# paulffm/Continuous-Time-Diffusion-Models-for-Discrete-Data

Measured on AMD Instinct MI355X. Metric: tau-leaping sample-steps/s, higher is better.
Workload: dtype bf16; 1 GPU; MNIST tauLDR U-Net TauL step (config_tauUnet_mnist: D=784, S=256, 1000-step grid); batch_per_gpu=256, global_batch=256, D=784, S=256, parallelism=sample-sharded x1, no collective in the loop

## Files before the change

### continuous-time-diffusion-models-for-discrete-data_amd/ctdd/native.py

```python
import ctypes as C
import os

import torch

_HERE = os.path.dirname(os.path.dirname(os.path.abspath(__file__)))
_LIB = None

BRANCH_CTELBO, BRANCH_CRM = 0, 1
LOGIT_TYPES = {"direct": 0, "reverse_prob": 1, "reverse_logscale": 2}
STEP_ORDINAL, STEP_CORRECTOR, STEP_COUNT_RAW, STEP_CRM, STEP_COUNT_JUMPS, STEP_BF16, STEP_LOGITS_BF16 = 1, 2, 4, 8, 16, 32, 64


class CtddError(RuntimeError):
    pass


def lib_path():
    return os.environ.get("CTDD_LIBRARY") or os.path.join(_HERE, "libctdd.so")


_P, _I, _F, _U64, _U32, _I64 = C.c_void_p, C.c_int, C.c_float, C.c_uint64, C.c_uint32, C.c_int64
_SIGS = {
    "ctdd_abi_version": ([], _I),
    "ctdd_last_error": ([], C.c_char_p),
    "ctdd_rate_table": ([_P, _P, _P, _P, _P, _P, _I, _I, _I, _F, _P, _P, _P, _P, _P], _I),
    "ctdd_noise_categorical": ([_P, _P, _P, _P, _U64, _U64, _I, _I, _I, _P, _P], _I),
    "ctdd_xtilde_sample": ([_P, _P, _P, _P, _P, _U64, _U64, _I, _I, _I, _P, _P, _P, _P], _I),
    "ctdd_xtilde_sample_masked": ([_P, _P, _P, _P, _P, _P, _U64, _U64, _I, _I, _I, _P, _P, _P, _P], _I),
    "ctdd_logprob": ([_P, _P, _P, _P, _I, _I, _I, _I, _P, _P, _P], _I),
    "ctdd_reverse_rates": ([_I, _I, _P, _P, _P, _P, _P, _F, _I, _I, _I, _P, _P, _P], _I),
    "ctdd_tauleap_apply": ([_P, _P, _P, _I, _I, _I, _I, _P, _P, _P], _I),
    "ctdd_tauleap_draw": ([_P, _P, _P, _F, _U32, _U64, _U64, _I, _I, _I, _P, _P, _P], _I),
    "ctdd_tauleap_step": ([_I, _I, _P, _P, _P, _P, _P, _F, _F, _F, _U32, _U64, _U64, _I, _I, _I, _P, _P, _P], _I),
    "ctdd_tauleap_step_rows": ([_I, _I, _P, _P, _P, _P, _P, _F, _F, _F, _U32, _U64, _U64, _I, _I, _I, _P, _I, _P, _P, _P], _I),
    "ctdd_lbjf_step": ([_I, _I, _P, _P, _P, _P, _F, _F, _F, _U32, _P, _U64, _U64, _I, _I, _I, _P, _P, _P, _P], _I),
    "ctdd_logprob_rp_mfma": ([_P, _P, _P, _I, _I, _I, _P, _P, _P, _P], _I),
    "ctdd_logprob_rp_bwd_mfma": ([_P, _P, _P, _P, _P, _F, _I, _I, _I, _P, _P, _P, _P, _P], _I),
    "ctdd_exact_step": ([_P, _P, _P, _P, _P, _U64, _U64, _I, _I, _I, _P, _P, _P, _P], _I),
    "ctdd_midpoint_predict": ([_I, _I, _P, _P, _P, _P, _F, _F, _F, _I, _I, _I, _P, _P], _I),
    "ctdd_lbjf_from_rates": ([_P, _P, _F, _P, _U64, _U64, _I, _I, _I, _P, _P, _P, _P], _I),
    "ctdd_midpoint_from_rates": ([_P, _P, _F, _I, _I, _I, _P, _P], _I),
    "ctdd_lbjf_step_rows": ([_I, _I, _P, _P, _P, _P, _F, _F, _F, _U32, _P, _U64, _U64, _I, _I, _I, _P, _I, _P, _P, _P, _P], _I),
    "ctdd_midpoint_predict_rows": ([_I, _I, _P, _P, _P, _P, _F, _F, _F, _I, _I, _I, _P, _I, _P, _P], _I),
    "ctdd_exact_step_rows": ([_P, _P, _P, _P, _P, _U64, _U64, _I, _I, _I, _P, _I, _P, _P, _P, _P], _I),
    "ctdd_lbjf_from_rates_rows": ([_P, _P, _F, _P, _U64, _U64, _I, _I, _I, _P, _I, _P, _P, _P, _P], _I),
    "ctdd_midpoint_from_rates_rows": ([_P, _P, _F, _I, _I, _I, _P, _I, _P, _P], _I),
    "ctdd_argmax": ([_P, _I, _I, _I, _P, _P], _I),
    "ctdd_initial_samples": ([_P, _U64, _U64, _I, _I, _I, _P, _P], _I),
    "ctdd_philox_uniform": ([_U64, _U64, _I64, _I, _P, _P], _I),
    "ctdd_s256_step_table_bytes": ([], _I64),
    "ctdd_s256_prepare": ([_P, _P, _F, _I, _P, _P, _P, _P], _I),
    "ctdd_s256_prepare_crm": ([_P, _P, _I, _P, _P, _P, _P], _I),
    "ctdd_tauleap_step_s256": ([_P, _P, _P, _P, _P, _P, _F, _F, _U32, _U64, _U64, _I, _I, _P, _P, _P, _P], _I),
    "ctdd_tauleap_step_s256_rows": ([_P, _P, _P, _P, _P, _P, _F, _F, _U32, _U64, _U64, _I, _I, _P, _I, _P, _P, _P, _P], _I),
    "ctdd_crm_loss": ([_P, _P, _P, _P, _I, _I, _I, _I, _F, _F, _P, _P, _P, _P], _I),
    "ctdd_ctelbo_scratch_bytes": ([_I, _I, _I], _I64),
    "ctdd_ctelbo_loss": ([_P, _P, _P, _P, _P, _P, _I, _I, _I, _F, _F, _F, _P, _P, _P, _P], _I),
    "ctdd_ctelbo_loss_terms": ([_P, _P, _P, _P, _P, _P, _I, _I, _I, _F, _F, _F, _F, _P, _P, _P, _P], _I),
    "ctdd_ctelbo_loss_window": ([_P, _P, _P, _P, _P, _P, _I, _I, _I, _I, _I, _F, _F, _F, _F, _P, _P, _P, _P], _I),
    "ctdd_ctelbo_loss_masked": ([_P, _P, _P, _P, _P, _P, _P, _I, _I, _I, _F, _F, _F, _F, _P, _P, _P, _P], _I),
    "ctdd_score_elbo_loss": ([_P, _P, _P, _P, _P, _P, _I, _I, _I, _F, _F, _P, _P, _P, _P], _I),
    "ctdd_crm_loss_ll": ([_P, _P, _P, _I, _I, _I, _I, _F, _P, _P, _P, _P], _I),
    "ctdd_score_elbo_loss_ll": ([_P, _P, _P, _P, _P, _P, _I, _I, _I, _F, _F, _P, _P, _P, _P], _I),
    "ctdd_logprob_bwd": ([_I, _P, _P, _P, _P, _P, _F, _I, _I, _I, _P, _P, _P, _P], _I),
    "ctdd_crm_loss_masked": ([_P, _P, _P, _P, _P, _I, _I, _I, _I, _F, _F, _P, _P, _P, _P], _I),
    "ctdd_crm_loss_ll_masked": ([_P, _P, _P, _P, _I, _I, _I, _I, _F, _P, _P, _P, _P], _I),
    "ctdd_score_elbo_loss_masked": ([_P, _P, _P, _P, _P, _P, _P, _I, _I, _I, _F, _F, _P, _P, _P, _P], _I),
    "ctdd_score_elbo_loss_ll_masked": ([_P, _P, _P, _P, _P, _P, _P, _I, _I, _I, _F, _F, _P, _P, _P, _P], _I),
    "ctdd_opt_chunk_elems": ([], _I),
    "ctdd_adam_ema_step": ([_P, _P, _I, _F, _F, _F, _F, _I64, _F, _F, _P, _P], _I),
    "ctdd_grad_sumsq": ([_P, _P, _I, _P, _I, _P], _I),
    "ctdd_adam_ema_apply": ([_P, _P, _I, _F, _F, _F, _F, _I64, _F, _F, _P, _P], _I),
}
UNET_EXPORTS = ("ctdd_unet_conv", "ctdd_unet_conv_patch", "ctdd_unet_conv_res", "ctdd_unet_conv_ring", "ctdd_unet_conv_up_phases", "ctdd_unet_upsample2x", "ctdd_unet_first_conv", "ctdd_unet_gn_apply", "ctdd_unet_gn_onepass", "ctdd_unet_channel_stats",
                "ctdd_unet_time", "ctdd_unet_time_uniform", "ctdd_unet_attention", "ctdd_unet_logistic_head", "ctdd_unet_resblock_small",
                "ctdd_unet_resblock_mid", "ctdd_unet_conv_rows")
HOLLOW_EXPORTS = ("ctdd_gemm_bf16", "ctdd_hollow_small_linear", "ctdd_hollow_embed", "ctdd_hollow_layernorm", "ctdd_hollow_add", "ctdd_hollow_put_rows", "ctdd_hollow_attention", "ctdd_hollow_attention_bf16")
UNET_TRAIN_EXPORTS = ("ctdd_unet_wgrad", "ctdd_unet_gn_bwd", "ctdd_unet_dropout", "ctdd_unet_colsum", "ctdd_unet_sum_batch", "ctdd_unet_sum_jobs", "ctdd_unet_accumulate",
                      "ctdd_unet_downsum2x", "ctdd_unet_upsample2x_f32", "ctdd_unet_cast_rows", "ctdd_unet_attention_bwd",
                      "ctdd_unet_first_conv_wgrad", "ctdd_unet_first_conv_wgrad_scratch", "ctdd_unet_pack_weights",
                      "ctdd_unet_unpack_grads")
HOLLOW_TRAIN_EXPORTS = ("ctdd_hollow_layernorm_bwd", "ctdd_hollow_attention_train", "ctdd_hollow_attention_bwd", "ctdd_hollow_attention_train_bf16", "ctdd_hollow_attention_bwd_bf16", "ctdd_hollow_act", "ctdd_hollow_relu_bf16", "ctdd_hollow_colsum", "ctdd_hollow_dropout",
                        "ctdd_hollow_embed_bwd")
BERT_EXPORTS = ("ctdd_bert_embed", "ctdd_bert_gather", "ctdd_bert_attention_short",
                "ctdd_bert_embed_bwd", "ctdd_bert_gather_bwd",
                "ctdd_bert_embed_enum_bwd", "ctdd_bert_gather_enum_bwd",
                "ctdd_bert_attention_short_train", "ctdd_bert_attention_short_bwd")
EXPORTS = tuple(_SIGS) + UNET_EXPORTS + HOLLOW_EXPORTS + UNET_TRAIN_EXPORTS + HOLLOW_TRAIN_EXPORTS + BERT_EXPORTS


def load():
    global _LIB
    if _LIB is None:
        path = lib_path()
        if not os.path.exists(path):
            raise CtddError(f"{path} not found: build it with `python __graft_entry__.py` "
                            "(hipcc --offload-arch=gfx950); there is no CPU fallback")
        lib = C.CDLL(path)
        for name, (argt, rest) in _SIGS.items():
            fn = getattr(lib, name)
            fn.argtypes, fn.restype = argt, rest
        _LIB = lib
    return _LIB


def _ptr(t, dtype=None, name="tensor"):
    if t is None:
        return None
    if not isinstance(t, torch.Tensor):
        raise CtddError(f"{name}: expected a torch tensor, got {type(t)}")
    if not t.is_cuda:
        raise CtddError(f"{name}: must live on a GPU (got {t.device}); libctdd has no CPU path")
    if dtype is not None and t.dtype != dtype:
        raise CtddError(f"{name}: expected {dtype}, got {t.dtype}")
    if not t.is_contiguous():
        raise CtddError(f"{name}: must be contiguous")
    return t.data_ptr()


def _stream():
    return torch.cuda.current_stream().cuda_stream


def _check(rc, what):
    if rc != 0:
        msg = load().ctdd_last_error().decode(errors="replace")
        raise CtddError(f"{what} failed with status {rc}: {msg}")


# ... 607 lines not shown
```

### continuous-time-diffusion-models-for-discrete-data_amd/ctdd/unet_engine.py

```python
import contextlib
import ctypes as C

import torch

from . import native
from .plan_launch import bound_launch, graph_capture, ptr

_P, _I, _F = C.c_void_p, C.c_int, C.c_float
SEG_3x3, SEG_1x1, SEG_3x3_S2, SEG_3x3_UP = 0, 1, 2, 3


class _Seg(C.Structure):
    _fields_ = [("hi", _P), ("f32", _P), ("C", _I), ("kind", _I)]


class _ConvArgs(C.Structure):
    _fields_ = [("seg", _Seg * 3), ("nseg", _I), ("w_hi", _P), ("w_f32", _P), ("B", _I), ("H", _I), ("W", _I),
                ("Hin", _I), ("Win", _I), ("N", _I), ("Ktot", _I), ("bias", _P), ("tbias", _P), ("tb_stride", _I),
                ("res_f32", _P), ("res_bf16", _P), ("out_f32", _P), ("out_hi", _P), ("stats", _P), ("logits_C", _I),
                ("ksplit", _I), ("acc_buf", _P), ("act", _I), ("out_lo", _P)]


class _FirstArgs(C.Structure):
    _fields_ = [("x64", _P), ("x32", _P), ("lo", _F), ("hi", _F), ("w", _P), ("bias", _P), ("B", _I), ("Cin", _I),
                ("H", _I), ("W", _I), ("Cout", _I), ("out_f32", _P), ("out_hi", _P), ("stats", _P), ("x0_f32", _P)]


class _GnArgs(C.Structure):
    _fields_ = [("s1_f32", _P), ("s1_bf16", _P), ("st1", _P), ("C1", _I), ("s2_f32", _P), ("s2_bf16", _P), ("st2", _P),
                ("C2", _I), ("gamma", _P), ("beta", _P), ("B", _I), ("HW", _I), ("G", _I), ("eps", _F), ("swish", _I),
                ("out_hi", _P), ("out_f32", _P)]


class _ResblockArgs(C.Structure):
    _fields_ = [("s1_bf16", _P), ("s2_bf16", _P), ("C1", _I), ("C2", _I), ("gamma1", _P), ("beta1", _P), ("gamma2", _P), ("beta2", _P),
                ("G1", _I), ("G2", _I), ("eps1", _F), ("eps2", _F), ("w1", _P), ("bias1", _P), ("tbias", _P), ("tb_stride", _I),
                ("w2", _P), ("bias2", _P), ("skip", _I), ("B", _I), ("H", _I), ("W", _I), ("N", _I), ("out_bf16", _P)]


class _ConvRowsArgs(C.Structure):
    _fields_ = [("s1_bf16", _P), ("st1", _P), ("C1", _I), ("s2_bf16", _P), ("st2", _P), ("C2", _I), ("gamma", _P), ("beta", _P), ("G", _I),
                ("eps", _F), ("w", _P), ("bias", _P), ("tbias", _P), ("tb_stride", _I), ("r1_bf16", _P), ("RC1", _I), ("r2_bf16", _P),
                ("RC2", _I), ("res_bf16", _P), ("out_bf16", _P), ("out_stats", _P), ("B", _I), ("H", _I), ("W", _I), ("N", _I)]


class _TimeArgs(C.Structure):
    _fields_ = [("t", _P), ("B", _I), ("ch", _I), ("tdim", _I), ("w1", _P), ("b1", _P), ("w2", _P), ("b2", _P),
                ("hid", _P), ("act", _P)]


class _AttnArgs(C.Structure):
    _fields_ = [("qkv", _P), ("B", _I), ("T", _I), ("C", _I), ("heads", _I), ("out_hi", _P), ("out_f32", _P)]


class _LogisticArgs(C.Structure):
    _fields_ = [("net", _P), ("x0", _P), ("B", _I), ("C", _I), ("HW", _I), ("S", _I), ("fix", _I), ("out", _P), ("fast", _I), ("out_bf16", _P)]


_sigs_done = False


def _lib():
    global _sigs_done
    lib = native.load()
    if not _sigs_done:
        for name, argt in (("ctdd_unet_conv", [_P, _I, _I, _I, _P]), ("ctdd_unet_conv_patch", [_P, _I, _I, _I, _P]), ("ctdd_unet_conv_res", [_P, _I, _P]), ("ctdd_unet_conv_ring", [_P, _I, _P]),
                           ("ctdd_unet_conv_up_phases", [_P, _I, _P]), ("ctdd_unet_upsample2x", [_P, _I, _I, _I, _I, _P, _P]), ("ctdd_unet_first_conv", [_P, _P]),
                           ("ctdd_unet_gn_apply", [_P, _P]), ("ctdd_unet_gn_onepass", [_P, _I, _I, _P]), ("ctdd_unet_channel_stats", [_P, _I, _I, _I, _P, _P]),
                           ("ctdd_unet_time", [_P, _P, _P, _I, _P, _P]), ("ctdd_unet_time_uniform", [_P, _P, _P, _I, _P, _P]),
                           ("ctdd_unet_attention", [_P, _P]), ("ctdd_unet_resblock_small", [_P, _I, _P]),
                           ("ctdd_unet_resblock_mid", [_P, _I, _P]), ("ctdd_unet_conv_rows", [_P, _I, _P]),
                           ("ctdd_unet_logistic_head", [_P, _P])):
            fn = getattr(lib, name)
            fn.argtypes, fn.restype = argt, _I
        _sigs_done = True
    return lib


def _unwrap(net):
    return net.module if hasattr(net, "module") and net.__class__.__name__ == "DistributedDataParallel" else net


def supports(model):
    net = _unwrap(getattr(model, "net", None))
    return (net is not None and net.__class__.__name__ == "UNet" and not model.padding
            and model.cfg.model.model_output in ("logits", "logistic_pars"))


def training_supported(model):
    if getattr(model.cfg.model, "engine_train", "hip") != "hip" or not supports(model):
        return False
    net = _unwrap(model.net)
    return net.channel % 16 == 0 and all((net.channel * int(m_)) % 16 == 0 for m_ in model.cfg.model.ch_mult)



def resblock_small_covers(H, W, cs, cout, G1, G2):
    Ct = sum(cs)
    if H * W > 64 or W > 8 or cout != 192 or len(cs) > 2 or any(c % 64 for c in cs) or Ct > 384 or Ct % G1 or cout % G2:
        return False
    if H * W > 16 and (H - 1) * (W + 2) + W > 80:
        return False
    rs_a, rs_2, prows = Ct * 2 + 32, cout * 2 + 32, (H + 2) * (W + 2)
    return H * W * rs_a + prows * max(rs_a, rs_2) + 256 * 80 + 2 * 384 * 8 + 2 * 384 * 4 <= 160 * 1024


def pack_resblock_weights(w2d):
    N, K = w2d.shape
    assert N == 192 and K % 64 == 0
    return w2d.reshape(4, 3, 16, K // 64, 2, 4, 8).permute(0, 3, 1, 4, 5, 2, 6).contiguous().reshape(N, K)


def resblock_mid_covers(H, W, cs, cout, G1, G2):
    Ct = sum(cs)
    if (H < 1 or W < 1 or H > 14 or W > 14 or cout != 192 or not 1 <= len(cs) <= 2
            or any(c <= 0 or c % 32 or c > 192 for c in cs) or G1 <= 0 or G2 <= 0 or Ct % G1 or cout % G2):
        return False
    return ((H + 2) * 16 + 2) * (cout * 2 + 32) + 256 * 80 + 2 * 384 * 8 + 2 * 384 * 4 <= 160 * 1024


def pack_row_tile_weights(w, cs, rcs, streams):
    N, Ct, Rt = w.shape[0], sum(cs), sum(rcs)
    assert N == 48 * streams and w.shape[1] == 9 * Ct + Rt and all(c % 32 == 0 for c in [*cs, *rcs])
    w3, parts, c0 = w[:, :9 * Ct].reshape(N, 9, Ct), [], 0
    for c in cs:
        v = w3[:, :, c0:c0 + c].reshape(streams, 3, 16, 3, 3, c // 32, 4, 8)
        parts.append(v.permute(0, 5, 4, 3, 1, 6, 2, 7).reshape(streams, -1))
        c0 += c
    c0 = 9 * Ct
    for c in rcs:
        v = w[:, c0:c0 + c].reshape(streams, 3, 16, c // 32, 4, 8)
        parts.append(v.permute(0, 3, 1, 4, 2, 5).reshape(streams, -1))
        c0 += c
    return torch.cat(parts, 1).contiguous().reshape(N, w.shape[1])


def pack_resblock_mid_weights(w1, w2, cs):
    N = w1.shape[0]
    return pack_row_tile_weights(w1, cs, [], 4), pack_row_tile_weights(w2, [N], cs if w2.shape[1] > 9 * N else [], 4)


def pack_conv_rows_weights(w, cs, rcs):
    return pack_row_tile_weights(w, cs, rcs, 2)


CONV_ROWS_MIN_WGS = 96


def conv_rows_covers(H, W, cs, rcs, cout, G, residual=False):
    return bool(H >= 1 and 1 <= W <= 28 and cout == 96 and 1 <= len(cs) <= 2 and len(rcs) <= 2 and all(c > 0 and c % 32 == 0 for c in [*cs, *rcs])
                and sum(cs) <= 384 and sum(rcs) <= 384 and G > 0 and sum(cs) % G == 0 and not (rcs and residual))


def fold_upsample_weights(w):
    N, Cn = w.shape[:2]
    assert tuple(w.shape[2:]) == (3, 3)
    sel = torch.tensor([[[1, 0, 0], [0, 1, 1]], [[1, 1, 0], [0, 0, 1]]], dtype=w.dtype, device=w.device)
    return torch.einsum("pia,qjb,ncab->pqnijc", sel, sel, w).reshape(4, N, 4 * Cn).contiguous()


def upsample_phases_covers(B, Hs, Ws, Cn, N):
    return bool(Cn >= 16 and Cn % 16 == 0 and (N % 96 == 0 or N % 64 == 0) and N > 0 and 1 <= Ws <= 33 and Hs * Ws >= 32
                and 4 * Cn * 64 < 2 ** 31 and 4 * B * Hs * Ws < 2 ** 31)


def _onepass_slab(B, HW, Cn, G, max_threads=1024):
    if Cn % 8 or G <= 0 or Cn % G:
        return 0
    cg = Cn // G
    L = cg
    while L % 8:
        L += cg
    best = 0
    for sc in range(L, Cn + 1, L):
        if Cn % sc:
            continue
        noct = sc // 8
        if noct > max_threads:
            continue
        npl = min(max_threads // noct, HW)
        if -(-HW // npl) > 12:
            continue
        wgs = B * (Cn // sc)
        if best == 0 or wgs >= 256:
            best = sc
        if wgs < 256:
            break
    return best


class _Tensor:

    def __init__(self, pb, H, W, Cn, stats=True):
        eng, B = pb.eng, pb.B
        M = B * H * W
        self.B, self.H, self.W, self.C = B, H, W, Cn
        self.f32 = torch.empty((M, Cn), dtype=torch.float32, device=eng.dev) if eng.precise else None
        self.hi = None if eng.precise else torch.empty((M, Cn), dtype=torch.bfloat16, device=eng.dev)
        small = H * W <= pb.no_stats_hw
        self.stats_by_gn = bool(stats and small and pb.gn_writes_stats)
        self.stats = pb.alloc_stats(B * Cn * 2) if (stats and (not small or self.stats_by_gn)) else None
        pb.keep.append(self)


# ... 160 lines not shown
        s1 = srcs[0]
        a.s1_f32, a.s1_bf16, a.C1 = (ptr(s1.f32), None, s1.C) if eng.precise else (None, ptr(s1.hi), s1.C)
        if s1.stats is not None:
            self.stats_views.append((a, s1.stats, "st1"))
        if len(srcs) == 2:
            s2 = srcs[1]
            a.s2_f32, a.s2_bf16, a.C2 = (ptr(s2.f32), None, s2.C) if eng.precise else (None, ptr(s2.hi), s2.C)
            if s2.stats is not None:
                self.stats_views.append((a, s2.stats, "st2"))
        g, b_ = norm.weight.detach().float().contiguous(), norm.bias.detach().float().contiguous()
        self.keep.extend([g, b_, a, out])
        a.gamma, a.beta = ptr(g), ptr(b_)
        a.B, a.HW, a.G, a.eps, a.swish = B, HW, norm.num_groups, eps, int(swish)
        a.out_hi, a.out_f32 = ptr(out.hi), ptr(out.f32)
        if self.onepass_gn and HW <= self.no_stats_hw:
            if _onepass_slab(B, HW, Ct, norm.num_groups, self.gn_threads) == 0:
                raise native.CtddError(f"one-pass GroupNorm does not cover HW={HW} C={Ct} G={norm.num_groups}")
            self.launch(lib.ctdd_unet_gn_onepass, C.byref(a), 0, self.gn_threads, label=f"gn1 {srcs[0].H}x{srcs[0].W} C={Ct} ({len(srcs)} src)")
        else:
            self.launch(lib.ctdd_unet_gn_apply, C.byref(a), label=f"gn {srcs[0].H}x{srcs[0].W} C={Ct} ({len(srcs)} src)")
        if tc is not None:
            tc.record_gn(self, srcs, norm, swish, eps, HW, out, drop_p)
        return out

    def conv_rows(self, srcs, norm, segs, wsrc, bias, out, tb=None, res=None, raws=()):
        eng, lib, B = self.eng, self.lib, self.B
        Hc, Wc, N = srcs[0].H, srcs[0].W, out.C
        cs, rcs = [s_.C for s_ in srcs], [s_.C for s_ in raws]
        a = _ConvRowsArgs()
        for i, s_ in enumerate(srcs):
            setattr(a, f"s{i + 1}_bf16", ptr(s_.hi))
            setattr(a, f"C{i + 1}", s_.C)
            self.stats_views.append((a, s_.stats, f"st{i + 1}"))
        for i, s_ in enumerate(raws):
            setattr(a, f"r{i + 1}_bf16", ptr(s_.hi))
            setattr(a, f"RC{i + 1}", s_.C)
        g, b_ = norm.weight.detach().float().contiguous(), norm.bias.detach().float().contiguous()
        a.gamma, a.beta, a.G, a.eps = ptr(g), ptr(b_), norm.num_groups, norm.eps
        w, _ = eng._pack(pack_conv_rows_weights(eng._w2d(wsrc, segs), cs, rcs))
        a.w, a.bias = ptr(w), ptr(bias)
        if tb is not None:
            a.tbias, a.tb_stride = tb
        if res is not None:
            a.res_bf16 = ptr(res.hi)
        a.out_bf16 = ptr(out.hi)
        if out.stats is not None and not out.stats_by_gn:
            self.stats_views.append((a, out.stats, "out_stats"))
        a.B, a.H, a.W, a.N = B, Hc, Wc, N
        self.keep.extend([g, b_, w, bias, a])
        Ktot = w.shape[1]
        self.launch(lib.ctdd_unet_conv_rows, C.byref(a), 0, label=f"{Hc}x{Wc} K={Ktot} N={N} gn+conv rows C={cs} raw={rcs}",
                    flops=2 * B * Hc * Wc * N * Ktot)

    def conv2_operands(self, rb, a2, srcs):
        tc = self.tc
        segs, wsrc, bias_params = [(a2, rb.conv2.weight.shape[0], SEG_3x3)], [(rb.conv2.weight, 0)], [rb.conv2.bias]
        bias = rb.conv2.bias.detach().float()
        if rb.skip is not None:
            c_ = 0
            for s_ in srcs:
                segs.append((s_, s_.C, SEG_1x1))
                wsrc.append((rb.skip.weight, c_))
                c_ += s_.C
            bias_params.append(rb.skip.bias)
            bias = tc.summed_bias(bias_params) if tc is not None else bias + rb.skip.bias.detach().float()
        return segs, wsrc, bias_params, bias.contiguous()

    def resblock_fused(self, rb, srcs, mid=False):
        eng, lib, B = self.eng, self.lib, self.B
        Hc, Wc = srcs[0].H, srcs[0].W
        cs = [s.C for s in srcs]
        Ct, cout = sum(cs), rb.conv1.weight.shape[0]
        y = _Tensor(self, Hc, Wc, cout)
        a = _ResblockArgs()
        a.s1_bf16, a.C1 = ptr(srcs[0].hi), cs[0]
        if len(srcs) == 2:
            a.s2_bf16, a.C2 = ptr(srcs[1].hi), cs[1]
        par = [p_.detach().float().contiguous() for p_ in (rb.norm1.weight, rb.norm1.bias, rb.norm2.weight, rb.norm2.bias, rb.conv1.bias)]
        a.gamma1, a.beta1, a.gamma2, a.beta2, a.bias1 = (ptr(p_) for p_ in par)
        a.G1, a.G2, a.eps1, a.eps2 = rb.norm1.num_groups, rb.norm2.num_groups, rb.norm1.eps, rb.norm2.eps
        a.tbias, a.tb_stride = self.tproj.data_ptr() + 4 * self.toff[id(rb)], self.tb_stride
        w1 = eng._w2d([(rb.conv1.weight, 0)], [(None, Ct, SEG_3x3)])
        segs, wsrc, _, bias2 = self.conv2_operands(rb, None, srcs)
        w2 = eng._w2d(wsrc, segs)
        w1, w2 = pack_resblock_mid_weights(w1, w2, cs) if mid else (pack_resblock_weights(w1), pack_resblock_weights(w2))
        (w1, _), (w2, _) = eng._pack(w1), eng._pack(w2)
        a.w1, a.w2, a.bias2, a.skip = ptr(w1), ptr(w2), ptr(bias2), int(rb.skip is not None)
        a.B, a.H, a.W, a.N, a.out_bf16 = B, Hc, Wc, cout, ptr(y.hi)
        self.keep.extend(par + [w1, w2, bias2, a])
        K1, K2 = w1.shape[1], w2.shape[1]
        self.launch(lib.ctdd_unet_resblock_mid if mid else lib.ctdd_unet_resblock_small, C.byref(a), 0,
                    label=f"{Hc}x{Wc} resblock C={cs} N={cout} K={K1}+{K2}", flops=2 * B * Hc * Wc * cout * (9 * Ct + 9 * cout + (Ct if rb.skip is not None else 0)))
        return y

    def resblock(self, rb, srcs):
        eng, tc = self.eng, self.tc
        Hc, Wc = srcs[0].H, srcs[0].W
        cs = [s.C for s in srcs]
        cout = rb.conv1.weight.shape[0]
        if self.onepass_gn and eng._fuses_resblock(rb, Hc, Wc, cs, tc is not None) and all(s_.stats is None for s_ in srcs):
            return self.resblock_fused(rb, srcs)
        if self.onepass_gn and eng._fuses_resblock_mid(rb, Hc, Wc, cs, tc is not None) and all(s_.stats is None for s_ in srcs):
            return self.resblock_fused(rb, srcs, mid=True)
        tbias = (self.tproj.data_ptr() + 4 * self.toff[id(rb)], self.tb_stride)
        h = _Tensor(self, Hc, Wc, cout)
        b1 = rb.conv1.bias.detach().float().contiguous()
# ... 96 lines not shown
        self.conv([(cur, cur.C, SEG_3x3_S2)], [(cv.weight, 0)],
                  cv.bias.detach().float().contiguous(), cur.C, Ho, Wo, cur.H, cur.W, y, bias_params=[cv.bias])
        return y

    def upsample_in_phases(self, cur):
        eng, m, B, Cn = self.eng, self.m, self.B, cur.C
        if self.tc is not None or eng.precise or not int(getattr(m, "upsample_phases", 1)):
            return False
        Ho, Wo = cur.H * 2, cur.W * 2
        ring = self.pick_kernel(True, B * Ho * Wo, Cn, Ho, Wo) == "ring" and Wo <= 33 and Cn % 32 == 0
        if not ring or (getattr(m, "conv_ksplit", 1) > 1 and Cn // 16 >= 2) or getattr(m, "ring_small_tiles", 0):
            return False
        return upsample_phases_covers(B, cur.H, cur.W, Cn, Cn)

    def upsample_phases(self, cv, cur, y):
        eng, B, Cn = self.eng, self.B, cur.C
        a = _ConvArgs()
        a.nseg = 1
        a.seg[0].hi, a.seg[0].C, a.seg[0].kind = ptr(cur.hi), Cn, SEG_3x3_UP
        whi, _ = eng._pack(fold_upsample_weights(cv.weight.detach().float()).reshape(4 * Cn, 4 * Cn))
        bias = cv.bias.detach().float().contiguous()
        a.w_hi, a.bias = ptr(whi), ptr(bias)
        a.B, a.H, a.W, a.Hin, a.Win, a.N, a.Ktot = B, y.H, y.W, cur.H, cur.W, Cn, 4 * Cn
        a.out_hi = ptr(y.hi)
        if y.stats is not None and not y.stats_by_gn:
            self.stats_views.append((a, y.stats, "stats"))
        self.keep.extend([whi, bias, a])
        self.launch(self.lib.ctdd_unet_conv_up_phases, C.byref(a), 0, label=f"{y.H}x{y.W} K=4x{4 * Cn} N={Cn} up-phases of {cur.H}x{cur.W}",
                    flops=2 * B * y.H * y.W * Cn * 4 * Cn)

    def upsample(self, cv, cur):
        eng, tc, B, lib = self.eng, self.tc, self.B, self.lib
        y = _Tensor(self, cur.H * 2, cur.W * 2, cur.C)
        if self.upsample_in_phases(cur):
            self.upsample_phases(cv, cur, y)
        elif eng.precise and tc is None:
            self.conv([(cur, cur.C, SEG_3x3_UP)], [(cv.weight, 0)],
                      cv.bias.detach().float().contiguous(), cur.C, cur.H * 2, cur.W * 2, cur.H, cur.W, y)
        else:
            up = _Tensor(self, cur.H * 2, cur.W * 2, cur.C, stats=False)
            if eng.precise:
                self.launch(lib.ctdd_unet_upsample2x_f32, ptr(cur.f32), B, cur.H, cur.W, cur.C, ptr(up.f32))
            else:
                self.launch(lib.ctdd_unet_upsample2x, ptr(cur.hi), B, cur.H, cur.W, cur.C, ptr(up.hi))
            if tc is not None:
                tc.record_upsample(cur, up)
            self.conv([(up, cur.C, SEG_3x3)], [(cv.weight, 0)],
                      cv.bias.detach().float().contiguous(), cur.C, up.H, up.W, up.H, up.W, y, bias_params=[cv.bias])
        return y

    def head(self, cur, logits_out, logits_bf16):
        eng, tc, B, st, m, net, dev, (Cin, H0, W0) = self.eng, self.tc, self.B, self.st, self.m, self.net, self.dev, self.shape
        S = net.S
        ao = self.gn_apply([cur], net.out[0], True, net.out[0].eps, cur.H * cur.W)
        oc = net.out[2]
        n_out = oc.weight.shape[0]
        D = Cin * H0 * W0
        logistic = m.model_output == "logistic_pars"
        ldt = torch.bfloat16 if logits_bf16 and not (logistic and (tc is not None or eng.precise or S % 4)) else torch.float32
        st.logits = logits_out if logits_out is not None else torch.empty((B, D, S), dtype=ldt, device=dev)
        assert st.logits.dtype == ldt
        if logistic:
            st.net_out = torch.empty((B * H0 * W0, n_out), dtype=torch.float32, device=dev)
            self.conv([(ao, ao.C, SEG_3x3)], [(oc.weight, 0)],
                      oc.bias.detach().float().contiguous(), n_out, H0, W0, H0, W0, None, out_f32_tensor=st.net_out, bias_params=[oc.bias])
            la = _LogisticArgs()
            la.net, la.x0, la.B, la.C, la.HW, la.S, la.fix = ptr(st.net_out), ptr(st.x0), B, Cin, H0 * W0, S, int(bool(m.fix_logistic))
            if ldt == torch.bfloat16:
                la.out_bf16 = ptr(st.logits)
            else:
                la.out = ptr(st.logits)
            la.fast = 0 if eng.precise else 1
            self.keep.append(la)
            if tc is None:
                self.launch(self.lib.ctdd_unet_logistic_head, C.byref(la))
        else:
            self.conv([(ao, ao.C, SEG_3x3)], [(oc.weight, 0)],
                      oc.bias.detach().float().contiguous(), n_out, H0, W0, H0, W0, None, out_f32_tensor=st.logits,
                      logits_C=Cin, bias_params=[oc.bias])

    def build(self, x_dtype, logits_out, logits_bf16, uniform_t):
        st, B, net, dev = self.st, self.B, self.net, self.dev
        st.x_in = torch.zeros((B, *self.shape), dtype=x_dtype, device=dev)
        st.t_in = torch.zeros((B,), dtype=torch.float32, device=dev)
        self.time(uniform_t)
        cur = self.first_conv(net.down[0])
        feats = [cur]
        for layer in list(net.down)[1:]:
            cur = self.block(layer, [cur]) if hasattr(layer, "resblocks") else self.downsample(layer.downsample[0], cur)
            feats.append(cur)
        for layer in net.mid:
            cur = self.block(layer, [cur])
        for layer in net.up:
            cur = self.block(layer, [cur, feats.pop()]) if hasattr(layer, "resblocks") else self.upsample(layer[1], cur)
        self.head(cur, logits_out, logits_bf16)
        if self.tc is not None:
            self.tc.finish(self)
        st.stats = torch.zeros((max(self.stats_off, 1),), dtype=torch.float64, device=dev)
        base = st.stats.data_ptr()
        for a_, off, field in self.stats_views:
            setattr(a_, field, base + 8 * off)
        nz = sum(n for _, n in self.zero_views)
        st.zpool = torch.zeros((max(nz, 1),), dtype=torch.float32, device=dev)
        zo = 0
        for a_, n in self.zero_views:
            a_.acc_buf = st.zpool.data_ptr() + 4 * zo
            zo += n
        st.plan, st.keep, st.graph = self.plan, self.keep, None
        return st


class UNetEngine:
    def __init__(self, model, precision=None):
        self.model = model
# ... 11 lines not shown
        self._time_w = None

    def _weights_version(self):
        return sum(p._version for p in self.net.parameters()) + 7919 * getattr(self.model, "_weights_version", 0)

    def _pack(self, w2d):
        w = w2d.detach().float().contiguous()
        return (None, w) if self.precise else (w.to(torch.bfloat16).contiguous(), None)

    @staticmethod
    def _w2d(wsrc, segs):
        parts = []
        for (w, c_off), (_, cs, kind) in zip(wsrc, segs):
            w = w.detach().float()
            N = w.shape[0]
            if kind == SEG_1x1:
                parts.append(w.reshape(N, -1)[:, c_off:c_off + cs])
            else:
                parts.append(w[:, c_off:c_off + cs].permute(0, 2, 3, 1).reshape(N, 9 * cs))
        return torch.cat(parts, dim=1).contiguous()


    def _time_weights(self):
        ver = self._weights_version()
        if self._time_w is None or self._time_w[0] != ver:
            net = self.net
            resblocks = [mod.resblocks for mod in list(net.down) + list(net.mid) + list(net.up) if hasattr(mod, "resblocks")]
            pw = torch.cat([rb.time[1].weight.detach().float() for rb in resblocks], 0).t().contiguous()
            pb = torch.cat([rb.time[1].bias.detach().float() for rb in resblocks], 0).contiguous()
            tw = [net.time[1].weight.t(), net.time[1].bias, net.time[3].weight.t(), net.time[3].bias]
            tw = [w.detach().float().contiguous() for w in tw]
            self._time_w = (ver, resblocks, pw, pb, tw)
        return self._time_w[1:]

    def _onepass_max_hw(self):
        return int(getattr(self.cfg.model, "gn_onepass_max_hw", 256))

    def _fuses_resblock(self, rb, Hc, Wc, cs, training):
        return bool(not training and not self.precise and int(getattr(self.cfg.model, "resblock_fused", 1))
                    and Hc * Wc <= self._onepass_max_hw()
                    and resblock_small_covers(Hc, Wc, cs, rb.conv1.weight.shape[0], rb.norm1.num_groups, rb.norm2.num_groups))

    def _fuses_resblock_mid(self, rb, Hc, Wc, cs, training):
        return bool(not training and not self.precise and int(getattr(self.cfg.model, "resblock_fused_mid", 1))
                    and Hc * Wc <= self._onepass_max_hw()
                    and not resblock_small_covers(Hc, Wc, cs, rb.conv1.weight.shape[0], rb.norm1.num_groups, rb.norm2.num_groups)
                    and resblock_mid_covers(Hc, Wc, cs, rb.conv1.weight.shape[0], rb.norm1.num_groups, rb.norm2.num_groups))

    def _runs_conv_rows(self, B, Hc, Wc, cs, rcs, cout, G, residual, training):
        m = self.cfg.model
        return bool(not training and not self.precise and int(getattr(m, "conv_rows", 1))
                    and conv_rows_covers(Hc, Wc, cs, rcs, cout, G, residual)
                    and B * -(-Hc // 14) >= int(getattr(m, "conv_rows_min_wgs", CONV_ROWS_MIN_WGS)))

    def _onepass_gn_covers(self, B, training):
        net, (_, H, W) = self.net, self.cfg.data.shape
        max_hw, threads = self._onepass_max_hw(), int(getattr(self.cfg.model, "gn_threads", 512))
        norms, c = [], net.channel
        for layer in [*list(net.down)[1:], *net.mid, *net.up]:
            if hasattr(layer, "downsample"):
                H, W = (H + 1 - 3) // 2 + 1, (W + 1 - 3) // 2 + 1
            elif not hasattr(layer, "resblocks"):
                H, W = 2 * H, 2 * W
            else:
                rb, c1 = layer.resblocks, layer.resblocks.norm1.num_channels
                cs = [c] if c1 == c else [c, c1 - c]
                if not (self._fuses_resblock(rb, H, W, cs, training) or self._fuses_resblock_mid(rb, H, W, cs, training)):
                    norms += [(H * W, rb.norm1), (H * W, rb.norm2)]
                c = rb.norm2.num_channels
                if layer.attention is not None:
                    norms.append((H * W, layer.attention.norm))
        norms.append((H * W, net.out[0]))
        return all(hw > max_hw or _onepass_slab(B, hw, n.num_channels, n.num_groups, threads) > 0 for hw, n in norms)

    def _build(self, B, x_dtype, logits_out=None, tc=None, logits_bf16=False, uniform_t=False):
        m = self.cfg.model
        onepass_gn = bool((not self.precise) and int(getattr(m, "gn_onepass", 1)) and (tc is None or int(getattr(m, "gn_onepass_train", 1)))
                          and self._onepass_gn_covers(B, tc is not None))
        return _PlanBuilder(self, B, tc, onepass_gn).build(x_dtype, logits_out, logits_bf16, uniform_t)

    def _run_plan(self, st):
        st.stats.zero_()
        st.zpool.zero_()
        for step in st.plan:
            step()

    def _prepare(self, B, x_dtype, x, times, logits_out=None, logits_bf16=False, uniform_t=False, time_row=None):
        st = self._build(B, x_dtype, logits_out, logits_bf16=logits_bf16, uniform_t=uniform_t)
        st.x_in.copy_(x.reshape(st.x_in.shape))
        self._set_time(st, times, time_row)
        self._run_plan(st)
        torch.cuda.synchronize()
        (st.graph,) = self._capture([lambda: self._run_plan(st)], "", "the plan runs as eager launches")
        return st

    def _capture(self, runs, what, then):
        if getattr(self.cfg.model, "engine_graph", True):
            try:
                graphs = []
                for run in runs:
                    graphs.append(torch.cuda.CUDAGraph())
                    with graph_capture(graphs[-1]):
                        run()
                return graphs
            except native.CtddError:
                raise
# ... 186 lines not shown
```

### include/ctdd_unet.h

```cpp
#ifndef CTDD_UNET_H
#define CTDD_UNET_H
#include <stdint.h>
#ifdef __cplusplus
extern "C" {
#endif

#define CTDD_SEG_3x3 0
#define CTDD_SEG_1x1 1
#define CTDD_SEG_3x3_S2 2
#define CTDD_SEG_3x3_UP 3
#define CTDD_SEG_3x3_S2T 4

typedef struct { const void* hi; const float* f32; int C, kind; } ctdd_conv_seg;
typedef struct {
  ctdd_conv_seg seg[3]; int nseg;
  const void* w_hi; const float* w_f32;
  int B, H, W, Hin, Win, N, Ktot;
  const float* bias; const float* tbias; int tb_stride;
  const float* res_f32; const void* res_bf16;
  float* out_f32; void* out_hi; double* stats; int logits_C;
  int ksplit; float* acc_buf;
  int act;
  void* out_lo;
} ctdd_conv_args;
int ctdd_unet_conv(const void* conv_args, int bk, int bnt, int f32, void* stream);
int ctdd_unet_conv_patch(const void* conv_args, int bk, int bnt, int wm, void* stream);
int ctdd_unet_conv_res(const void* conv_args, int bnt, void* stream);
int ctdd_unet_conv_ring(const void* conv_args, int bnt, void* stream);
int ctdd_unet_conv_up_phases(const void* conv_args, int f32, void* stream);
int ctdd_unet_upsample2x(const void* x_bf16,int B, int H, int W, int C, void* out_bf16, void* stream);

typedef struct {
  const int64_t* x64; const int32_t* x32; float lo, hi; const float* w; const float* bias;
  int B, Cin, H, W, Cout; float* out_f32; void* out_hi; double* stats; float* x0_f32;
} ctdd_first_conv_args;
int ctdd_unet_first_conv(const void* first_conv_args, void* stream);

typedef struct {
  const float* s1_f32; const void* s1_bf16; const double* st1; int C1;
  const float* s2_f32; const void* s2_bf16; const double* st2; int C2;
  const float* gamma; const float* beta; int B, HW, G; float eps; int swish; void* out_hi; float* out_f32;
} ctdd_gn_args;
int ctdd_unet_gn_apply(const void* gn_args, void* stream);
int ctdd_unet_gn_onepass(const void* gn_args, int slab_channels, int max_threads, void* stream);
int ctdd_unet_channel_stats(const float* x, int B, int HW, int C, double* stats, void* stream);

typedef struct {
  const void* s1_bf16; const void* s2_bf16; int C1, C2;
  const float* gamma1; const float* beta1; const float* gamma2; const float* beta2; int G1, G2; float eps1, eps2;
  const void* w1; const float* bias1; const float* tbias; int tb_stride;
  const void* w2; const float* bias2;
  int skip;
  int B, H, W, N; void* out_bf16;
} ctdd_resblock_args;
int ctdd_unet_resblock_small(const void* resblock_args, int f32, void* stream);
int ctdd_unet_resblock_mid(const void* resblock_args, int f32, void* stream);

typedef struct {
  const void* s1_bf16; const double* st1; int C1;
  const void* s2_bf16; const double* st2; int C2;
  const float* gamma; const float* beta; int G; float eps;
  const void* w; const float* bias; const float* tbias; int tb_stride;
  const void* r1_bf16; int RC1; const void* r2_bf16; int RC2;
  const void* res_bf16;
  void* out_bf16; double* out_stats;
  int B, H, W, N;
} ctdd_conv_rows_args;
int ctdd_unet_conv_rows(const void* conv_rows_args, int f32, void* stream);

typedef struct {
  const float* t; int B, ch, tdim;
  const float* w1; const float* b1; const float* w2; const float* b2;
  float* hid; float* act;
} ctdd_time_args;
int ctdd_unet_time(const void* time_args, const float* proj_w, const float* proj_b, int Ntot, float* proj_out, void* stream);
int ctdd_unet_time_uniform(const void* time_args, const float* proj_w, const float* proj_b, int Ntot, float* proj_out, void* stream);

typedef struct { const float* qkv; int B, T, C, heads; void* out_hi; float* out_f32; } ctdd_attn_args;
int ctdd_unet_attention(const void* attn_args, void* stream);

typedef struct { const float* net; const float* x0; int B, C, HW, S, fix; float* out;
                 int fast;
                 void* out_bf16;    } ctdd_logistic_args;
int ctdd_unet_logistic_head(const void* logistic_args, void* stream);

#ifdef __cplusplus
}
#endif
#endif
```

Before: 125,700 sample-steps/s.

## Fuse output GroupNorm+swish into the head 3x3 conv with a row-band kernel

Adds a dedicated kernel that computes GroupNorm scale and shift from precomputed statistics, applies norm+swish while filling an LDS slab of 14-row bands, then runs the final 3x3 conv to the 256-logit output in multiple 96-channel passes and stores bf16 logits directly. This replaces the separate gn_apply pass and generic conv for the direct-logit head, removing an intermediate activation round-trip and a launch. It is gated on bf16 logits, a single input channel, inference mode and enough workgroups. With B=256 and a 28x28 grid that gives 512 workgroups, each with one large LDS allocation, so occupancy and pass count may limit the gain.

```diff
diff --git a/continuous-time-diffusion-models-for-discrete-data_amd/csrc/unet_head_kernels.hip b/continuous-time-diffusion-models-for-discrete-data_amd/csrc/unet_head_kernels.hip
--- /dev/null
+++ b/continuous-time-diffusion-models-for-discrete-data_amd/csrc/unet_head_kernels.hip
@@ -0,0 +1,215 @@
+#include "row_tile.hpp"
+#include "../../include/ctdd_unet.h"
+
+namespace ctdd {
+namespace {
+
+constexpr int HD_THREADS = 256, HD_TILE = 96, HD_BAND = 14, HD_PITCH = 32, HD_RS = 224, HD_MAXW = 28, HD_MAXC = 96, HD_MAXN = 576;
+constexpr int HD_SLAB = ((HD_BAND + 2) * HD_PITCH + 2) * HD_RS;
+constexpr int HD_SCALE = HD_SLAB;
+constexpr int HD_STAGE = HD_SCALE + 2 * HD_MAXC * 4;
+constexpr int HD_SROWS = HD_BAND / 2, HD_WSTAGE = HD_SROWS * 16 * 96;
+constexpr int HD_TOTAL = HD_STAGE + 4 * HD_WSTAGE;
+constexpr unsigned HD_OOB = 0x80000000u;
+constexpr int HD_FB = 12;
+static_assert(HD_TOTAL <= 160 * 1024 && HD_STAGE % 16 == 0 && HD_BAND % 2 == 0, "slab + scale / shift + staging within the CU's LDS");
+
+__device__ __attribute__((always_inline)) inline void hd_fill(unsigned char* sm, const unsigned short* __restrict__ src, int cs, int pc, int coff,
+                                                             int y0, int H, int W) {
+  const int t = threadIdx.x, noct = pc >> 3, npl = HD_THREADS / noct;
+  if (t >= noct * npl) return;
+  const int oct = t % noct, pl = t / noct;
+  const float* scale = (const float*)(sm + HD_SCALE) + coff + oct * 8;
+  const float* shift = scale + HD_MAXC;
+  const float4 sc0 = *(const float4*)scale, sc1 = *(const float4*)(scale + 4);
+  const float4 sh0 = *(const float4*)shift, sh1 = *(const float4*)(shift + 4);
+  const f32x2v scv[4] = {{sc0.x, sc0.y}, {sc0.z, sc0.w}, {sc1.x, sc1.y}, {sc1.z, sc1.w}};
+  const f32x2v shv[4] = {{sh0.x, sh0.y}, {sh0.z, sh0.w}, {sh1.x, sh1.y}, {sh1.z, sh1.w}};
+  const int rlo = y0 == 0 ? 1 : 0, rhi = H - y0 < HD_BAND + 1 ? H - y0 : HD_BAND + 1;
+  const unsigned npix = (unsigned)((rhi - rlo + 1) * W), uW = (unsigned)W;
+  const unsigned short* sp = src + (size_t)((y0 - 1 + rlo) * W) * cs + oct * 8;
+  unsigned char* dst = sm + (1 + rlo * HD_PITCH + 1) * HD_RS + oct * 16;
+  for (unsigned p0 = (unsigned)pl; p0 < npix; p0 += (unsigned)(HD_FB * npl)) {
+    u32x4 u[HD_FB];
+#pragma unroll
+    for (int k = 0; k < HD_FB; ++k) {
+      const unsigned p = p0 + (unsigned)(k * npl);
+      u[k] = *(const u32x4*)(sp + (size_t)(p < npix ? p : npix - 1) * cs);
+    }
+#pragma unroll
+    for (int k = 0; k < HD_FB; ++k) {
+      const unsigned p = p0 + (unsigned)(k * npl);
+      unsigned ow[4];
+#pragma unroll
+      for (int j = 0; j < 4; ++j) {
+        const f32x2v x = {__uint_as_float(u[k][j] << 16), __uint_as_float(u[k][j] & 0xFFFF0000u)};
+        f32x2v y = __builtin_elementwise_fma(x, scv[j], shv[j]);
+        const f32x2v z = y * (f32x2v){-1.4426950408889634f, -1.4426950408889634f};
+        const f32x2v d = (f32x2v){__builtin_amdgcn_exp2f(z.x), __builtin_amdgcn_exp2f(z.y)} + (f32x2v){1.0f, 1.0f};
+        y = y * (f32x2v){__builtin_amdgcn_rcpf(d.x), __builtin_amdgcn_rcpf(d.y)};
+        ow[j] = rt_pack2(y.x, y.y);
+      }
+      const unsigned rr = p / uW, x = p - rr * uW;
+      if (p < npix) *(uint4*)(dst + (rr * HD_PITCH + x) * HD_RS) = make_uint4(ow[0], ow[1], ow[2], ow[3]);
+    }
+  }
+}
+
+#ifdef CTDD_ROWS_STAMPS
+#define HD_STAMP(i_)                                                                                      \
+  do {                                                                                                    \
+    unsigned long long t_;                                                                                \
+    asm volatile("s_memtime %0\n\ts_waitcnt lgkmcnt(0)" : "=s"(t_)::"memory");                            \
+    if (threadIdx.x == 0) ((unsigned long long*)a.out_stats)[(size_t)blockIdx.x * 16 + (i_)] = t_;        \
+  } while (0)
+#else
+#define HD_STAMP(i_)
+#endif
+
+__global__ __launch_bounds__(HD_THREADS, 1) void k_conv_rows_head(const ctdd_conv_rows_args a) {
+  extern __shared__ __attribute__((aligned(16))) unsigned char sm[];
+  const int t = threadIdx.x;
+  const int H = a.H, W = a.W, HW = H * W, C1 = a.C1, N = a.N;
+  const int nbands = (H + HD_BAND - 1) / HD_BAND;
+  const int b = blockIdx.x / nbands, y0 = (blockIdx.x - b * nbands) * HD_BAND;
+  const int wv = __builtin_amdgcn_readfirstlane(t >> 6), cg = wv >> 1, hh = wv & 1;
+  const int nu3 = 3 * (C1 >> 5), npass = (N + HD_TILE - 1) / HD_TILE;
+  const size_t wstream = (size_t)nu3 * RT_UNIT;
+  const unsigned short* wcg = (const unsigned short*)a.w + (size_t)cg * wstream;
+  const unsigned short* wrow = wcg + (t & 63) * 8;
+  u32x4 wr[2][3][3];
+  HD_STAMP(0);
+
+  rt_wload9(wr[0], wrow, 0);
+  rt_wload9(wr[1], wrow, 1);
+  for (int v = t; v < (HD_SLAB >> 4); v += HD_THREADS) *(uint4*)(sm + v * 16) = make_uint4(0, 0, 0, 0);
+  {
+    float* scale = (float*)(sm + HD_SCALE);
+    float* shift = scale + HD_MAXC;
+    const int cgp = C1 / a.G;
+    for (int c = t; c < C1; c += HD_THREADS) {
+      const int g0 = (c / cgp) * cgp;
+      double s = 0.0, q = 0.0;
+      for (int j = g0; j < g0 + cgp; ++j) {
+        const double* st = a.st1 + ((size_t)b * C1 + j) * 2;
+        s += st[0]; q += st[1];
+      }
+      const double n = (double)cgp * (double)HW;
+      const double mean = s / n;
+      const double var = fmax(q / n - mean * mean, 0.0);
+      const float rstd = (float)(1.0 / sqrt(var + (double)a.eps));
+      scale[c] = rstd * a.gamma[c];
+      shift[c] = a.beta[c] - (float)mean * rstd * a.gamma[c];
+    }
+  }
+  __syncthreads();
+  HD_STAMP(1);
+
+  hd_fill(sm, (const unsigned short*)a.s1_bf16 + (size_t)b * HW * C1, C1, C1, 0, y0, H, W);
+  __syncthreads();
+  HD_STAMP(2);
+
+  const int nrows = H - y0 < HD_BAND ? H - y0 : HD_BAND;
+  unsigned char* stg = sm + HD_STAGE + wv * HD_WSTAGE;
+  unsigned short* outb = (unsigned short*)a.out_bf16 + ((size_t)b * HW + (size_t)y0 * W) * N;
+  const __amdgpu_buffer_rsrc_t orsrc = __builtin_amdgcn_make_buffer_rsrc((void*)outb, 0, nrows * W * N * 2, 0x00020000);
+
+  for (int p = 0; p < npass; ++p) {
+    const int lk = rt_again(t) & 63;
+    const int fb = (1 + 16 * hh + (lk & 15)) * HD_RS + (lk >> 4) * 16;
+    const unsigned short* wrow = wcg + lk * 8;
+    f32x4 acc[3][HD_BAND];
+#pragma unroll
+    for (int tt = 0; tt < 3; ++tt)
+#pragma unroll
+      for (int y = 0; y < HD_BAND; ++y) acc[tt][y] = (f32x4){0.0f, 0.0f, 0.0f, 0.0f};
+#pragma unroll
+    for (int tt = 0; tt < 3; ++tt)
+#pragma unroll
+      for (int y = 0; y < HD_BAND; ++y) asm volatile("" : "+a"(acc[tt][y]));
+    rt_gemm_rows<true, HD_RS, HD_PITCH>(acc, wr, wrow + (size_t)(2 * p) * wstream, nu3, sm, fb, HD_BAND);
+#pragma unroll
+    for (int tt = 0; tt < 3; ++tt)
+#pragma unroll
+      for (int y = 0; y < HD_BAND; ++y) asm volatile("" : "+a"(acc[tt][y]));
+    if (p + 1 < npass) {
+      rt_wload9(wr[0], wrow + (size_t)(2 * p + 2) * wstream, 0);
+      rt_wload9(wr[1], wrow + (size_t)(2 * p + 2) * wstream, 1);
+    }
+    HD_STAMP(3 + 2 * p);
+
+    const int n0 = p * HD_TILE + cg * 48;
+    const int lane = rt_again(t) & 63, lj = lane & 15, lq = lane >> 4;
+    const int nre = rt_again(nrows), We = rt_again(W);
+    float add[3][4];
+#pragma unroll
+    for (int tt = 0; tt < 3; ++tt) {
+      const int n = n0 + tt * 16 + lq * 4;
+      const float4 bv = n < N ? *(const float4*)(a.bias + n) : make_float4(0.0f, 0.0f, 0.0f, 0.0f);
+      add[tt][0] = bv.x; add[tt][1] = bv.y; add[tt][2] = bv.z; add[tt][3] = bv.w;
+    }
+#pragma unroll
+    for (int half = 0; half < 2; ++half) {
+#pragma unroll
+      for (int r = 0; r < HD_SROWS; ++r)
+#pragma unroll
+        for (int tt = 0; tt < 3; ++tt) {
+          const f32x4 v = acc[tt][half * HD_SROWS + r];
+          *(uint2*)(stg + (r * 16 + lj) * 96 + tt * 32 + lq * 8) =
+              make_uint2(rt_pack2(v[0] + add[tt][0], v[1] + add[tt][1]), rt_pack2(v[2] + add[tt][2], v[3] + add[tt][3]));
+        }
+      __builtin_amdgcn_fence(__ATOMIC_RELEASE, "wavefront");
+      __builtin_amdgcn_wave_barrier();
+      constexpr int NV = HD_SROWS * 16 * 6, NK = (NV + 63) / 64;
+      uint4 o[NK];
+#pragma unroll
+      for (int k = 0; k < NK; ++k) o[k] = *(const uint4*)(stg + (lane + 64 * k < NV ? lane + 64 * k : NV - 1) * 16);
+#pragma unroll
+      for (int k = 0; k < NK; ++k) {
+        const int v = lane + 64 * k, pi = v / 6, c8 = (v - pi * 6) * 8, y = half * HD_SROWS + (pi >> 4), col = 16 * hh + (pi & 15);
+        const bool ok = v < NV && y < nre && col >= 1 && col <= We && n0 + c8 < N;
+        __builtin_amdgcn_raw_buffer_store_b128(__builtin_bit_cast(u32x4, o[k]), orsrc, ok ? (unsigned)(((y * We + col - 1) * N + n0 + c8) * 2) : HD_OOB, 0, 0);
+      }
+      __builtin_amdgcn_fence(__ATOMIC_ACQ_REL, "wavefront");
+      __builtin_amdgcn_wave_barrier();
+    }
+    HD_STAMP(4 + 2 * p);
+  }
+}
+
+}
+}
+
+using namespace ctdd;
+
+extern "C" int ctdd_unet_conv_rows_head(const void* args_, int f32, void* stream) {
+  CTDD_REQUIRE(args_, CTDD_EINVAL, "ctdd_unet_conv_rows_head: null arguments");
+  const ctdd_conv_rows_args& a = *(const ctdd_conv_rows_args*)args_;
+  CTDD_REQUIRE(f32 == 0, CTDD_ERANGE, "ctdd_unet_conv_rows_head: bf16 inference only (the fp32 mode keeps GroupNorm and convolution apart)");
+  CTDD_REQUIRE(a.B > 0 && a.H > 0 && a.W >= 1 && a.W <= HD_MAXW, CTDD_ERANGE,
+               "ctdd_unet_conv_rows_head: a grid of %dx%d pixels does not fit the row tiles (1 <= W <= 28)", a.H, a.W);
+  const int nbands = (a.H + HD_BAND - 1) / HD_BAND;
+  CTDD_REQUIRE((int64_t)a.B * nbands < ((int64_t)1 << 31) && (int64_t)a.H * a.W * HD_MAXN < ((int64_t)1 << 30), CTDD_ERANGE,
+               "ctdd_unet_conv_rows_head: B=%d, %dx%d is over the 32-bit index range of the kernel", a.B, a.H, a.W);
+  CTDD_REQUIRE((a.C1 == 32 || a.C1 == 64 || a.C1 == 96) && a.C2 == 0 && a.RC1 == 0 && a.RC2 == 0 && a.N >= 32 && a.N <= HD_MAXN && a.N % 32 == 0,
+               CTDD_ERANGE,
+               "ctdd_unet_conv_rows_head: channel counts off the tile (N=%d, C1=%d, C2=%d, RC1=%d, RC2=%d; one source of 32, 64 or 96 channels, "
+               "N in multiples of 32 from 32 to 576)", a.N, a.C1, a.C2, a.RC1, a.RC2);
+  CTDD_REQUIRE(a.G > 0 && a.C1 % a.G == 0, CTDD_EINVAL, "ctdd_unet_conv_rows_head: %d groups do not divide %d channels", a.G, a.C1);
+  CTDD_REQUIRE(a.s1_bf16 && a.gamma && a.beta && a.w && a.bias && a.out_bf16, CTDD_EINVAL, "ctdd_unet_conv_rows_head: null pointer");
+  CTDD_REQUIRE(a.st1, CTDD_EINVAL, "ctdd_unet_conv_rows_head: a GroupNorm source without statistics");
+#ifdef CTDD_ROWS_STAMPS
+  const bool no_stats = true;
+#else
+  const bool no_stats = !a.out_stats;
+#endif
+  CTDD_REQUIRE(!a.res_bf16 && !a.tbias && no_stats, CTDD_EINVAL,
+               "ctdd_unet_conv_rows_head: the head takes no residual, time bias or output statistics");
+  auto al16 = [](const void* p) { return ((uintptr_t)p & 15) == 0; };
+  CTDD_REQUIRE(al16(a.s1_bf16) && al16(a.w) && al16(a.out_bf16) && al16(a.bias), CTDD_EINVAL,
+               "ctdd_unet_conv_rows_head: tensors must be 16-byte aligned");
+  static bool attr_done[16] = {};
+  ensure_lds_ceiling((const void*)k_conv_rows_head, attr_done);
+  hipLaunchKernelGGL(k_conv_rows_head, dim3(a.B * nbands), dim3(HD_THREADS), (size_t)HD_TOTAL, (hipStream_t)stream, a);
+  return finish_launch("k_conv_rows_head");
+}
diff --git a/continuous-time-diffusion-models-for-discrete-data_amd/ctdd/native.py b/continuous-time-diffusion-models-for-discrete-data_amd/ctdd/native.py
--- a/continuous-time-diffusion-models-for-discrete-data_amd/ctdd/native.py
+++ b/continuous-time-diffusion-models-for-discrete-data_amd/ctdd/native.py
@@ -74,7 +74,7 @@
 }
 UNET_EXPORTS = ("ctdd_unet_conv", "ctdd_unet_conv_patch", "ctdd_unet_conv_res", "ctdd_unet_conv_ring", "ctdd_unet_conv_up_phases", "ctdd_unet_upsample2x", "ctdd_unet_first_conv", "ctdd_unet_gn_apply", "ctdd_unet_gn_onepass", "ctdd_unet_channel_stats",
                 "ctdd_unet_time", "ctdd_unet_time_uniform", "ctdd_unet_attention", "ctdd_unet_logistic_head", "ctdd_unet_resblock_small",
-                "ctdd_unet_resblock_mid", "ctdd_unet_conv_rows")
+                "ctdd_unet_resblock_mid", "ctdd_unet_conv_rows", "ctdd_unet_conv_rows_head")
 HOLLOW_EXPORTS = ("ctdd_gemm_bf16", "ctdd_hollow_small_linear", "ctdd_hollow_embed", "ctdd_hollow_layernorm", "ctdd_hollow_add", "ctdd_hollow_put_rows", "ctdd_hollow_attention", "ctdd_hollow_attention_bf16")
 UNET_TRAIN_EXPORTS = ("ctdd_unet_wgrad", "ctdd_unet_gn_bwd", "ctdd_unet_dropout", "ctdd_unet_colsum", "ctdd_unet_sum_batch", "ctdd_unet_sum_jobs", "ctdd_unet_accumulate",
                       "ctdd_unet_downsum2x", "ctdd_unet_upsample2x_f32", "ctdd_unet_cast_rows", "ctdd_unet_attention_bwd",
diff --git a/continuous-time-diffusion-models-for-discrete-data_amd/ctdd/unet_engine.py b/continuous-time-diffusion-models-for-discrete-data_amd/ctdd/unet_engine.py
--- a/continuous-time-diffusion-models-for-discrete-data_amd/ctdd/unet_engine.py
+++ b/continuous-time-diffusion-models-for-discrete-data_amd/ctdd/unet_engine.py
@@ -70,6 +70,7 @@
                            ("ctdd_unet_time", [_P, _P, _P, _I, _P, _P]), ("ctdd_unet_time_uniform", [_P, _P, _P, _I, _P, _P]),
                            ("ctdd_unet_attention", [_P, _P]), ("ctdd_unet_resblock_small", [_P, _I, _P]),
                            ("ctdd_unet_resblock_mid", [_P, _I, _P]), ("ctdd_unet_conv_rows", [_P, _I, _P]),
+                           ("ctdd_unet_conv_rows_head", [_P, _I, _P]),
                            ("ctdd_unet_logistic_head", [_P, _P])):
             fn = getattr(lib, name)
             fn.argtypes, fn.restype = argt, _I
@@ -150,6 +151,20 @@
 def conv_rows_covers(H, W, cs, rcs, cout, G, residual=False):
     return bool(H >= 1 and 1 <= W <= 28 and cout == 96 and 1 <= len(cs) <= 2 and len(rcs) <= 2 and all(c > 0 and c % 32 == 0 for c in [*cs, *rcs])
                 and sum(cs) <= 384 and sum(rcs) <= 384 and G > 0 and sum(cs) % G == 0 and not (rcs and residual))
+
+
+def pack_conv_rows_head_weights(w, C1):
+    N, passes = w.shape[0], -(-w.shape[0] // 96)
+    wp = torch.zeros((96 * passes, w.shape[1]), dtype=w.dtype, device=w.device)
+    wp[:N] = w
+    return pack_row_tile_weights(wp, [C1], [], 2 * passes)
+
+
+HEAD_ROWS_MIN_WGS = 192
+
+
+def conv_rows_head_covers(H, W, C1, N, G):
+    return bool(H >= 1 and 1 <= W <= 28 and C1 in (32, 64, 96) and G > 0 and C1 % G == 0 and 32 <= N <= 576 and N % 32 == 0)
 
 
 def fold_upsample_weights(w):
@@ -416,6 +431,22 @@
         self.launch(lib.ctdd_unet_conv_rows, C.byref(a), 0, label=f"{Hc}x{Wc} K={Ktot} N={N} gn+conv rows C={cs} raw={rcs}",
                     flops=2 * B * Hc * Wc * N * Ktot)
 
+    def conv_rows_head(self, src, norm, oc, logits):
+        eng, B = self.eng, self.B
+        N, C1 = oc.weight.shape[0], src.C
+        a = _ConvRowsArgs()
+        a.s1_bf16, a.C1 = ptr(src.hi), C1
+        self.stats_views.append((a, src.stats, "st1"))
+        g, b_ = norm.weight.detach().float().contiguous(), norm.bias.detach().float().contiguous()
+        a.gamma, a.beta, a.G, a.eps = ptr(g), ptr(b_), norm.num_groups, norm.eps
+        w, _ = eng._pack(pack_conv_rows_head_weights(eng._w2d([(oc.weight, 0)], [(None, C1, SEG_3x3)]), C1))
+        bias = oc.bias.detach().float().contiguous()
+        a.w, a.bias, a.out_bf16 = ptr(w), ptr(bias), ptr(logits)
+        a.B, a.H, a.W, a.N = B, src.H, src.W, N
+        self.keep.extend([g, b_, w, bias, a])
+        self.launch(self.lib.ctdd_unet_conv_rows_head, C.byref(a), 0, label=f"{src.H}x{src.W} K={9 * C1} N={N} gn+conv rows head C={[C1]}",
+                    flops=2 * B * src.H * src.W * N * 9 * C1)
+
     def conv2_operands(self, rb, a2, srcs):
         tc = self.tc
         segs, wsrc, bias_params = [(a2, rb.conv2.weight.shape[0], SEG_3x3)], [(rb.conv2.weight, 0)], [rb.conv2.bias]
@@ -618,7 +649,6 @@
     def head(self, cur, logits_out, logits_bf16):
         eng, tc, B, st, m, net, dev, (Cin, H0, W0) = self.eng, self.tc, self.B, self.st, self.m, self.net, self.dev, self.shape
         S = net.S
-        ao = self.gn_apply([cur], net.out[0], True, net.out[0].eps, cur.H * cur.W)
         oc = net.out[2]
         n_out = oc.weight.shape[0]
         D = Cin * H0 * W0
@@ -626,6 +656,11 @@
         ldt = torch.bfloat16 if logits_bf16 and not (logistic and (tc is not None or eng.precise or S % 4)) else torch.float32
         st.logits = logits_out if logits_out is not None else torch.empty((B, D, S), dtype=ldt, device=dev)
         assert st.logits.dtype == ldt
+        if (not logistic and Cin == 1 and ldt == torch.bfloat16 and cur.stats is not None
+                and eng._runs_head_rows(B, cur.H, cur.W, cur.C, n_out, net.out[0].num_groups, tc is not None)):
+            self.conv_rows_head(cur, net.out[0], oc, st.logits)
+            return
+        ao = self.gn_apply([cur], net.out[0], True, net.out[0].eps, cur.H * cur.W)
         if logistic:
             st.net_out = torch.empty((B * H0 * W0, n_out), dtype=torch.float32, device=dev)
             self.conv([(ao, ao.C, SEG_3x3)], [(oc.weight, 0)],
@@ -743,6 +778,12 @@
         return bool(not training and not self.precise and int(getattr(m, "conv_rows", 1))
                     and conv_rows_covers(Hc, Wc, cs, rcs, cout, G, residual)
                     and B * -(-Hc // 14) >= int(getattr(m, "conv_rows_min_wgs", CONV_ROWS_MIN_WGS)))
+
+    def _runs_head_rows(self, B, Hc, Wc, C1, N, G, training):
+        m = self.cfg.model
+        return bool(not training and not self.precise and int(getattr(m, "conv_rows", 1)) and int(getattr(m, "head_rows", 1))
+                    and conv_rows_head_covers(Hc, Wc, C1, N, G)
+                    and B * -(-Hc // 14) >= int(getattr(m, "head_rows_min_wgs", HEAD_ROWS_MIN_WGS)))
 
     def _onepass_gn_covers(self, B, training):
         net, (_, H, W) = self.net, self.cfg.data.shape
diff --git a/include/ctdd_unet.h b/include/ctdd_unet.h
--- a/include/ctdd_unet.h
+++ b/include/ctdd_unet.h
@@ -67,6 +67,7 @@
   int B, H, W, N;
 } ctdd_conv_rows_args;
 int ctdd_unet_conv_rows(const void* conv_rows_args, int f32, void* stream);
+int ctdd_unet_conv_rows_head(const void* conv_rows_args, int f32, void* stream);
 
 typedef struct {
   const float* t; int B, ch, tdim;
```

New measurement: 129,900 sample-steps/s, median of 6. 3.3% higher.
